# stella-cv/stella_vslam

Measured on NVIDIA H100. Metric: frames/sec (ORB+match+local BA) @1920x1080, 2000 kpts, higher is better.
Workload: dtype u8

## Files before the change

### stella_vslam_b200/csrc/lba_kernels.cu

```cuda
#include <algorithm>
#include <cmath>
#include <cstdlib>
#include <new>
#include <sched.h>

#include <chrono>
#include <memory>
#include <mutex>
#include <thread>
#include <vector>

#include "common.cuh"
#include "lm_common.cuh"
#include "quat.cuh"
#include "staging.cuh"
#include "track_chain.cuh"

namespace b200 {
namespace lba {

constexpr double kPi = 3.14159265358979323846;

struct Cam {
    int model;
// ... 302 lines not shown
        for (int j = lane; j < i; j += 32) s += W.pose_cnt[j];
#pragma unroll
        for (int d = 16; d > 0; d >>= 1) s += __shfl_down_sync(0xFFFFFFFFu, s, d);
        if (lane == 0) {
            s_start = s;
            W.pose_start[i] = s;
            if (i == W.Kf - 1) W.pose_start[W.Kf] = s + W.pose_cnt[i];
        }
    }
    __syncthreads();
    int run = s_start;
    for (int base = 0; base < W.E; base += kListThreads) {
        const int s = base + tid;
        const bool mine = s < W.E && W.epcol[s] == i;
        const unsigned bal = __ballot_sync(0xFFFFFFFFu, mine);
        if (lane == 0) warp_cnt[warp] = __popc(bal);
        __syncthreads();
        int off = 0, tot = 0;
#pragma unroll
        for (int w2 = 0; w2 < kListThreads / 32; ++w2) {
            const int c = warp_cnt[w2];
            if (w2 < warp) off += c;
            tot += c;
        }
        if (mine) {
            const int slot = run + off + __popc(bal & ((1u << lane) - 1u));
            W.pose_edges[slot] = s;
            const EdgeS* ed = W.edges + s;
            const int l = ed->point, c_lo = W.pt_start[l];
            W.rowrec[slot] = make_int4(s, ed->lcol >= 0 ? l : -1, c_lo, W.pt_start[l + 1] - c_lo);
        }
        run += tot;
        __syncthreads();
    }
}

constexpr int kSchurChunk = 64;
struct SchurBlock {
    int i, j, chunk_start, chunk_end;
};
struct SchurChunk {
    int start, end, diag, block;
};
__device__ __forceinline__ void block_to_ij(int b, int Kf, int& i, int& j) {
    const double t = 2.0 * Kf + 1.0;
    i = (int)((t - sqrt(t * t - 8.0 * b)) * 0.5);
    i = max(0, min(i, Kf - 1));
    while (i > 0 && i * Kf - i * (i - 1) / 2 > b) --i;
    while (i + 1 < Kf && (i + 1) * Kf - (i + 1) * i / 2 <= b) ++i;
    j = i + (b - (i * Kf - i * (i - 1) / 2));
}
template <bool EMIT>
__global__ void __launch_bounds__(128) plan_pairs_kernel(const WinDev* __restrict__ wins) {
    const WinDev& W = wins[blockIdx.y];
    const int lane = threadIdx.x & 31, b = blockIdx.x * 4 + (threadIdx.x >> 5);
    if (b >= W.n_blocks || *W.bad_input) return;
    int i, j;
    block_to_ij(b, W.Kf, i, j);
    const int a_lo = W.pose_start[i], a_hi = W.pose_start[i + 1], mw = W.mask_words;
    int run = EMIT ? W.blk_pair_start[b] : 0;
    for (int base = a_lo; base < a_hi; base += 32) {
        const int pos = base + lane;
        bool hit = false;
        int4 rec = make_int4(0, -1, 0, 0);
        if (pos < a_hi) {
            rec = W.rowrec[pos];
            if (rec.y >= 0) hit = (W.lm_mask[(size_t)rec.y * mw + (j >> 6)] >> (j & 63)) & 1ull;
        }
        const unsigned bal = __ballot_sync(0xFFFFFFFFu, hit);
        if (EMIT && hit) {
            int c = rec.z;
            for (int q = 0; q < rec.w; ++q)
                if (W.epcol[rec.z + q] == j) {
                    c = rec.z + q;
                    break;
                }
            W.pairs[run + __popc(bal & ((1u << lane) - 1u))] = make_int4(rec.x, c, W.pt_col[rec.y], 0);
        }
        run += __popc(bal);
    }
    if (!EMIT) {
        if (lane == 0) W.blk_cnt[b] = run;
        return;
    }
    const int ps = W.blk_pair_start[b], total = W.blk_pair_start[b + 1] - ps, cs = W.blk_chunk_start[b];
    for (int ch = lane; ch * kSchurChunk < total; ch += 32)
        W.chunks[cs + ch] = SchurChunk{ps + ch * kSchurChunk, ps + min(total, (ch + 1) * kSchurChunk), i == j ? 1 : 0, b};
    if (lane == 0) W.blocks[b] = SchurBlock{i, j, cs, W.blk_chunk_start[b + 1]};
}
__global__ void __launch_bounds__(1024) plan_pair_scan_kernel(const WinDev* __restrict__ wins) {
    const WinDev& W = wins[blockIdx.x];
    if (*W.bad_input) return;
    __shared__ int ws_p[32], ws_c[32];
    const int tid = threadIdx.x, lane = tid & 31, warp = tid >> 5, nb = W.n_blocks;
    int carry_p = 0, carry_c = 0;
    for (int base = 0; base < nb; base += 1024) {
        const int b = base + tid;
        const int vp = b < nb ? W.blk_cnt[b] : 0, vc = ceil_div(vp, kSchurChunk);
        int xp = vp, xc = vc;
#pragma unroll
        for (int d = 1; d < 32; d <<= 1) {
            const int yp = __shfl_up_sync(0xFFFFFFFFu, xp, d), yc = __shfl_up_sync(0xFFFFFFFFu, xc, d);
            if (lane >= d) {
                xp += yp;
                xc += yc;
            }
        }
        if (lane == 31) {
            ws_p[warp] = xp;
            ws_c[warp] = xc;
        }
        __syncthreads();
        if (warp == 0) {
            int sp = ws_p[lane], sc = ws_c[lane];
#pragma unroll
            for (int d = 1; d < 32; d <<= 1) {
                const int yp = __shfl_up_sync(0xFFFFFFFFu, sp, d), yc = __shfl_up_sync(0xFFFFFFFFu, sc, d);
                if (lane >= d) {
                    sp += yp;
                    sc += yc;
                }
            }
            ws_p[lane] = sp;
            ws_c[lane] = sc;
        }
        __syncthreads();
        if (b < nb) {
            W.blk_pair_start[b] = carry_p + (warp ? ws_p[warp - 1] : 0) + xp - vp;
            W.blk_chunk_start[b] = carry_c + (warp ? ws_c[warp - 1] : 0) + xc - vc;
        }
        carry_p += ws_p[31];
        carry_c += ws_c[31];
        __syncthreads();
    }
    if (tid == 0) {
        W.blk_pair_start[nb] = carry_p;
        W.blk_chunk_start[nb] = carry_c;
    }
}

__device__ double ordered_sum(const double* __restrict__ p, int n, double* stage) {
    double s = 0.0;
    for (int base = 0; base < n; base += 1024) {
        const int m = min(1024, n - base);
        __syncthreads();
        for (int i = threadIdx.x; i < m; i += blockDim.x) stage[i] = __ldcg(p + base + i);
        __syncthreads();
        if (threadIdx.x == 0)
            for (int i = 0; i < m; ++i) s += stage[i];
    }
    return s;
}

__device__ void compute_dinv(const WinDev& W, double lambda) {
    const int Lf = W.Lf;
    const double* __restrict__ Hll = W.Hll;
    double* __restrict__ Dinv = W.Dinv;
    for (int lc = threadIdx.x; lc < Lf; lc += blockDim.x) {
        const double A0 = __ldcg(Hll + lc) + lambda, A1 = __ldcg(Hll + (size_t)Lf + lc), A2 = __ldcg(Hll + (size_t)2 * Lf + lc);
        const double A4 = __ldcg(Hll + (size_t)3 * Lf + lc) + lambda, A5 = __ldcg(Hll + (size_t)4 * Lf + lc), A8 = __ldcg(Hll + (size_t)5 * Lf + lc) + lambda;
        const double c0 = A4 * A8 - A5 * A5, c1 = A5 * A2 - A1 * A8, c2 = A1 * A5 - A4 * A2;
        const double det = A0 * c0 + A1 * c1 + A2 * c2;
        if (det == 0.0 || !isfinite(det)) {
            *W.fail = 1;
            continue;
        }
        const double id = 1.0 / det;
        Dinv[lc] = c0 * id;
        Dinv[(size_t)Lf + lc] = c1 * id;
        Dinv[(size_t)2 * Lf + lc] = c2 * id;
        Dinv[(size_t)3 * Lf + lc] = (A0 * A8 - A2 * A2) * id;
        Dinv[(size_t)4 * Lf + lc] = (A1 * A2 - A0 * A5) * id;
        Dinv[(size_t)5 * Lf + lc] = (A0 * A4 - A1 * A1) * id;
    }
}

__global__ void lm_round_begin_kernel(const WinDev* __restrict__ wins, int n_windows, int iterations, int round, double gain_thr) {
    const int w = blockIdx.x * blockDim.x + threadIdx.x;
    if (w >= n_windows) return;
    LmCtl* c = wins[w].ctl;
    c->round = round;
    c->iterations = iterations;
    c->gain_thr = gain_thr;
    c->iters_done[round] = 0;
    c->need_build = 1;
    if (*wins[w].bad_input) {
        c->skip_round2 = 1;
        c->outer_go = 0;
        return;
    }
    if (round == 1 && c->abort_word && lm_aborted(c)) {
        c->skip_round2 = 1;
        c->outer_go = 0;
        return;
    }
    c->stop_flag = 0;
    c->it = 0;
    c->ok = 1;
    c->outer_go = (iterations > 0 && !(c->abort_word && *c->abort_word)) ? 1 : 0;
}

__device__ void lm_after_build(const WinDev& W, double* stage) {
    LmCtl* c = W.ctl;
    const bool first = c->it == 0;
    double chi = 0.0;
    if (first) chi = ordered_sum(W.r_chi, W.lbc, stage);
    if (threadIdx.x == 0) {
        if (first) {
            c->current_chi = chi;
            double mx = 0.0;
            for (int i = 0; i < W.lbc; ++i) mx = fmax(mx, __ldcg(W.r_diag + i));
            for (int p = 0; p < W.Kf; ++p)
                for (int a = 0; a < 6; ++a) mx = fmax(mx, fabs(__ldcg(W.Hpp + 36 * (size_t)p + a * 7)));
            c->lambda = 1e-5 * mx;
            c->ni = 2.0;
            if (c->round == 0) c->lambda_init = c->lambda;
        }
        c->qmax = 0;
        c->rho = 0.0;
        c->need_build = 0;
        *W.fail = 0;
    }
    __syncthreads();
    compute_dinv(W, c->lambda);
}

__device__ void lm_after_trial(const WinDev& W, double* stage) {
    LmCtl* c = W.ctl;
    const double* r_result = W.r_result;
    const bool ok2 = __ldcg(r_result) != 0.0;
    const double chi_sum = ordered_sum(W.r_chi, W.lbc, stage);
    const double scale_sum = ordered_sum(W.r_scale, W.lbc, stage);
    __shared__ int s_again;
    if (threadIdx.x == 0) {
        c->trials += 1;
        const double temp_chi = ok2 ? chi_sum : 1.7976931348623157e308;
        double rho = c->current_chi - temp_chi;
        double scale = ok2 ? __ldcg(r_result + 1) + scale_sum : 0.0;
        scale += 1e-3;
        rho /= scale;
        bool broke = false;
        if (rho > 0 && isfinite(temp_chi) && ok2) {
            double alpha = 1. - pow(2 * rho - 1, 3.0);
            alpha = fmin(alpha, 2. / 3.);
            c->lambda *= fmax(1. / 3., alpha);
            c->ni = 2.0;
            c->current_chi = temp_chi;
            c->cur ^= 1;
        } else {
            c->lambda *= c->ni;
            c->ni *= 2.0;
            if (!isfinite(c->lambda)) broke = true;
        }
        if (!broke) c->qmax++;
        c->rho = rho;
        const bool again = !broke && rho < 0 && c->qmax < 10 && !lm_aborted(c);
        s_again = again ? 1 : 0;
        *W.fail = 0;
        if (!again) {
            if (c->qmax == 10 || rho == 0 || !isfinite(c->lambda)) c->ok = 0;
            const double chi_now = c->current_chi;
            if (c->it == 0) {
                c->last_chi = chi_now;
            } else {
                const double gain = (c->last_chi - chi_now) / chi_now;
                c->last_chi = chi_now;
                if (gain >= 0 && gain < c->gain_thr) c->stop_flag = 1;
            }
            c->chi2[c->round] = chi_now;
            c->lambda_final[c->round] = c->lambda;
            c->it++;
            c->iters_done[c->round] = c->it;
            c->need_build = 1;
            c->outer_go = (c->it < c->iterations && !lm_aborted(c) && c->ok) ? 1 : 0;
        }
    }
    __syncthreads();
    if (s_again) compute_dinv(W, c->lambda);
}

__device__ __forceinline__ bool last_cta_arrives(int* ticket, int n_ctas, int* smem_flag) {
    __threadfence();
    __syncthreads();
    if (threadIdx.x == 0) {
        const int t = atomicAdd(ticket, 1);
        *smem_flag = (t == n_ctas - 1);
        if (*smem_flag) *ticket = 0;
    }
    __syncthreads();
    const bool last = *smem_flag != 0;
    if (last) __threadfence();
    return last;
}

__global__ void __launch_bounds__(256) lm_round_end_kernel(const WinDev* __restrict__ wins, int round) {
    __shared__ double stage[1024];
    const WinDev& W = wins[blockIdx.x];
    LmCtl* c = W.ctl;
    if (*W.bad_input || (round == 1 && c->skip_round2)) return;
    const double chi = ordered_sum(W.r_chi, W.lbc, stage);
    if (threadIdx.x) return;
    if (c->iters_done[round] == 0) c->chi2[round] = chi;
}

enum { kBuild = 0, kTrial = 1, kRoundEnd = 2 };
constexpr int kLmThreads = 128;

template <int MODE>
__global__ void __launch_bounds__(kLmThreads, 4) landmark_kernel(const WinDev* __restrict__ wins) {
    __shared__ double sh[kLmThreads];
    const WinDev& W = wins[blockIdx.y];
    if ((int)blockIdx.x >= W.lbc) return;
    const LmCtl* ctl = W.ctl;
    if (MODE == kBuild && !(ctl->outer_go && ctl->need_build)) return;
    if (MODE == kTrial && !ctl->outer_go) return;
    if (MODE == kRoundEnd && (*W.bad_input || (ctl->round == 1 && ctl->skip_round2))) return;
    const int sidx = (ctl->cur ^ (MODE == kTrial ? 1 : 0)) & 1;
    const double* __restrict__ Rt = W.Rt[sidx];
    const double* __restrict__ pts = W.pts[sidx];
    double* __restrict__ chi = W.chi[sidx];
    const double* __restrict__ chi_carry = W.chi[sidx ^ 1];
    const int sub = threadIdx.x & 7;
    const int l = blockIdx.x * 16 + (threadIdx.x >> 3);
    const bool valid = l < W.L;
    const int a0 = valid ? W.pt_start[l] : 0, b0 = valid ? W.pt_start[l + 1] : 0;
    const int lc = valid ? W.pt_col[l] : -1;
    double cost = 0.0;
    double h[9] = {0, 0, 0, 0, 0, 0, 0, 0, 0};
    double P[3] = {0, 0, 0};
    if (valid) {
        P[0] = pts[3 * (size_t)l];
        P[1] = pts[3 * (size_t)l + 1];
        P[2] = pts[3 * (size_t)l + 2];
    }
    for (int e = a0 + sub; e < b0; e += 8) {
        const EdgeS ed = W.edges[e];
        double* __restrict__ rec = W.Hpl + (size_t)e * kHplStride;
        if (W.level[e] == 0) {
            const Cam c = W.cams[ed.cam];
            double err[3], pc[3];
            const double* T = Rt + 12 * (size_t)ed.pose;
            edge_residual(ed, c, T, P, err, pc);
            const double w = (double)ed.inv_sigma_sq;
            const double e2 = w * (err[0] * err[0] + err[1] * err[1] + err[2] * err[2]);
            chi[e] = e2;
            const bool rob = W.robust[e] != 0;
            cost += rob ? huber_cost(e2, (double)ed.delta) : e2;
            if (MODE == kBuild) {
                double Ji[9], Jj[18];
                edge_jacobians(ed, c, T, pc, Ji, Jj);
                const double ww = w * (rob ? huber_weight(e2, (double)ed.delta) : 1.0);
                const bool lfree = lc >= 0, pfree = ed.pcol >= 0;
                if (lfree) {
                    h[0] += ww * (Ji[0] * Ji[0] + Ji[3] * Ji[3] + Ji[6] * Ji[6]);
                    h[1] += ww * (Ji[0] * Ji[1] + Ji[3] * Ji[4] + Ji[6] * Ji[7]);
                    h[2] += ww * (Ji[0] * Ji[2] + Ji[3] * Ji[5] + Ji[6] * Ji[8]);
                    h[3] += ww * (Ji[1] * Ji[1] + Ji[4] * Ji[4] + Ji[7] * Ji[7]);
                    h[4] += ww * (Ji[1] * Ji[2] + Ji[4] * Ji[5] + Ji[7] * Ji[8]);
                    h[5] += ww * (Ji[2] * Ji[2] + Ji[5] * Ji[5] + Ji[8] * Ji[8]);
                    h[6] += -ww * (Ji[0] * err[0] + Ji[3] * err[1] + Ji[6] * err[2]);
                    h[7] += -ww * (Ji[1] * err[0] + Ji[4] * err[1] + Ji[7] * err[2]);
                    h[8] += -ww * (Ji[2] * err[0] + Ji[5] * err[1] + Ji[8] * err[2]);
                }
                const bool both = lfree && pfree;
                double hr[12];
#pragma unroll
                for (int a = 0; a < 3; ++a)
#pragma unroll
                    for (int b = 0; b < 3; ++b) {
                        const double s = ww * (Jj[3 + a] * Ji[b] + Jj[9 + a] * Ji[3 + b] + Jj[15 + a] * Ji[6 + b]);
                        hr[a * 3 + b] = both ? s : 0.0;
                    }
#pragma unroll
                for (int i = 0; i < 3; ++i) hr[9 + i] = both ? pc[i] : 0.0;
#pragma unroll
                for (int i = 0; i < 3; ++i) st256(rec + 4 * i, hr[4 * i], hr[4 * i + 1], hr[4 * i + 2], hr[4 * i + 3]);
            }
        } else if (MODE == kBuild) {
#pragma unroll
            for (int i = 0; i < 3; ++i) st256(rec + 4 * i, 0.0, 0.0, 0.0, 0.0);
        } else if (MODE == kTrial) {
            chi[e] = chi_carry[e];
        }
    }
    if (MODE == kBuild) {
#pragma unroll
        for (int i = 0; i < 9; ++i)
#pragma unroll
            for (int s = 4; s > 0; s >>= 1) h[i] += __shfl_down_sync(0xFFFFFFFFu, h[i], s, 8);
        double mx = 0.0;
        if (valid && sub == 0 && lc >= 0) {
            const int Lf = W.Lf;
#pragma unroll
            for (int i = 0; i < 6; ++i) W.Hll[(size_t)i * Lf + lc] = h[i];
#pragma unroll
            for (int i = 0; i < 3; ++i) W.bl[(size_t)i * Lf + lc] = h[6 + i];
            mx = fmax(fabs(h[0]), fmax(fabs(h[3]), fabs(h[5])));
        }
        sh[threadIdx.x] = mx;
        __syncthreads();
        for (int s = blockDim.x >> 1; s > 0; s >>= 1) {
            if (threadIdx.x < s) sh[threadIdx.x] = fmax(sh[threadIdx.x], sh[threadIdx.x + s]);
            __syncthreads();
        }
        if (threadIdx.x == 0) W.r_diag[blockIdx.x] = sh[0];
        __syncthreads();
    }
    const double s = block_sum(cost, sh);
    if (threadIdx.x == 0) W.r_chi[blockIdx.x] = s;
    if (MODE == kTrial) {
        __shared__ int last_flag;
        __shared__ double stage[1024];
        if (!last_cta_arrives(W.tickets + 1, W.lbc, &last_flag)) return;
        lm_after_trial(W, stage);
    }
}

constexpr int kRowThreads = 256;
__global__ void __launch_bounds__(kRowThreads) pose_rows_kernel(const WinDev* __restrict__ wins) {
    const WinDev& W = wins[blockIdx.y];
    const LmCtl* ctl = W.ctl;
    if (!(ctl->outer_go && ctl->need_build)) return;
    const int n_rows = max(W.Kf, 1);
    if ((int)blockIdx.x >= n_rows) return;
    __shared__ double part[kRowThreads / 32][27];
    __shared__ int last_flag;
    __shared__ double stage[1024];
    const int tid = threadIdx.x, lane = tid & 31, warp = tid >> 5;
    if ((int)blockIdx.x < W.Kf) {
        const int i = blockIdx.x;
        const double* __restrict__ Rt = W.Rt[ctl->cur & 1];
        const double* __restrict__ pts = W.pts[ctl->cur & 1];
        const int a = W.pose_start[i], b = W.pose_start[i + 1];
        const int per = round_up(ceil_div(max(b - a, 1), kRowThreads / 32), 32);
        const int lo = a + warp * per, hi = min(b, lo + per);
        double acc[27];
#pragma unroll
        for (int x = 0; x < 27; ++x) acc[x] = 0.0;
        for (int k = lo + lane; k < hi; k += 32) {
            const int e = W.pose_edges[k];
            if (W.level[e]) continue;
            const EdgeS ed = W.edges[e];
            const Cam c = W.cams[ed.cam];
            double err[3], pc[3], Ji[9], Jj[18];
            const double* T = Rt + 12 * (size_t)ed.pose;
            edge_residual(ed, c, T, pts + 3 * (size_t)ed.point, err, pc);
            edge_jacobians(ed, c, T, pc, Ji, Jj);
            const double w = (double)ed.inv_sigma_sq;
            const double e2 = w * (err[0] * err[0] + err[1] * err[1] + err[2] * err[2]);
            const double ww = w * (W.robust[e] ? huber_weight(e2, (double)ed.delta) : 1.0);
            int t = 0;
#pragma unroll
            for (int x = 0; x < 6; ++x)
#pragma unroll
                for (int y = x; y < 6; ++y) acc[t++] += ww * (Jj[x] * Jj[y] + Jj[6 + x] * Jj[6 + y] + Jj[12 + x] * Jj[12 + y]);
#pragma unroll
            for (int x = 0; x < 6; ++x) acc[21 + x] += -ww * (Jj[x] * err[0] + Jj[6 + x] * err[1] + Jj[12 + x] * err[2]);
        }
#pragma unroll
        for (int x = 0; x < 27; ++x)
#pragma unroll
            for (int s = 16; s > 0; s >>= 1) acc[x] += __shfl_down_sync(0xFFFFFFFFu, acc[x], s);
        if (lane == 0)
#pragma unroll
            for (int x = 0; x < 27; ++x) part[warp][x] = acc[x];
        __syncthreads();
        if (tid < 27) {
            double r = 0.0;
#pragma unroll
            for (int w2 = 0; w2 < kRowThreads / 32; ++w2) r += part[w2][tid];
            if (tid < 21) {
                int x = 0, rem = tid;
                while (rem >= 6 - x) {
                    rem -= 6 - x;
                    ++x;
                }
                const int y = x + rem;
                W.Hpp[(size_t)i * 36 + x * 6 + y] = r;
                W.Hpp[(size_t)i * 36 + y * 6 + x] = r;
            } else {
                W.bp[(size_t)i * 6 + (tid - 21)] = r;
            }
        }
    }
    if (!last_cta_arrives(W.tickets, n_rows, &last_flag)) return;
    lm_after_build(W, stage);
}

__device__ __forceinline__ void dmma_m8n8k4(double& c0, double& c1, double a, double b) {
    asm volatile("mma.sync.aligned.m8n8k4.row.col.f64.f64.f64.f64 {%0,%1}, {%2}, {%3}, {%0,%1};" : "+d"(c0), "+d"(c1) : "d"(a), "d"(b));
}

__device__ __forceinline__ void schur_finish_block(const WinDev& W, const SchurBlock sb, double lambda, int lane) {
    const double* __restrict__ partials = W.chunk_part;
    double* __restrict__ M = W.M;
    const int n = W.n, ld = W.ld;
    for (int el = lane; el < 42; el += 32) {
        if (el >= 36 && sb.i != sb.j) continue;
        double sacc = 0.0;
        for (int c = sb.chunk_start; c < sb.chunk_end; ++c) sacc += __ldcg(partials + (size_t)c * 42 + el);
        if (el < 36) {
            const int r = el / 6, c = el - r * 6;
            double val = -sacc;
            if (sb.i == sb.j) val += W.Hpp[(size_t)sb.i * 36 + el] + (r == c ? lambda : 0.0);
            M[(size_t)(6 * sb.j + c) * ld + 6 * sb.i + r] = val;
            if (sb.i == sb.j) M[(size_t)(6 * sb.i + r) * ld + 6 * sb.j + c] = val;
        } else {
            const int r = el - 36;
            M[(size_t)n * ld + 6 * sb.i + r] = W.bp[(size_t)sb.i * 6 + r] - sacc;
        }
    }
}

__device__ void se3_oplus(const double* q, const double* t, const double* upd, double* qo, double* to) {
    const double* om = upd;
    const double* up = upd + 3;
    const double theta = sqrt(om[0] * om[0] + om[1] * om[1] + om[2] * om[2]);
    const double O[9] = {0, -om[2], om[1], om[2], 0, -om[0], -om[1], om[0], 0};
    double O2[9];
    for (int i = 0; i < 3; ++i)
        for (int j = 0; j < 3; ++j) O2[i * 3 + j] = O[i * 3] * O[j] + O[i * 3 + 1] * O[3 + j] + O[i * 3 + 2] * O[6 + j];
    double a, b, c, d;
    if (theta < 0.00001) {
        a = 1.0; b = 0.5; c = 0.5; d = 1.0 / 6.0;
    } else {
        a = sin(theta) / theta;
        b = (1 - cos(theta)) / (theta * theta);
        c = b;
        d = (theta - sin(theta)) / (theta * theta * theta);
    }
    double R[9], V[9];
    for (int i = 0; i < 9; ++i) {
        const double I = (i % 4 == 0) ? 1.0 : 0.0;
        R[i] = I + a * O[i] + b * O2[i];
        V[i] = I + c * O[i] + d * O2[i];
    }
    double dq[4], dt[3];
    rot_to_quat(R, dq);
    quat_normalize(dq);
    for (int i = 0; i < 3; ++i) dt[i] = V[i * 3] * up[0] + V[i * 3 + 1] * up[1] + V[i * 3 + 2] * up[2];
    double uv[3] = {dq[1] * t[2] - dq[2] * t[1], dq[2] * t[0] - dq[0] * t[2], dq[0] * t[1] - dq[1] * t[0]};
    uv[0] += uv[0]; uv[1] += uv[1]; uv[2] += uv[2];
    to[0] = dt[0] + t[0] + dq[3] * uv[0] + (dq[1] * uv[2] - dq[2] * uv[1]);
    to[1] = dt[1] + t[1] + dq[3] * uv[1] + (dq[2] * uv[0] - dq[0] * uv[2]);
    to[2] = dt[2] + t[2] + dq[3] * uv[2] + (dq[0] * uv[1] - dq[1] * uv[0]);
    double nq[4];
    nq[3] = dq[3] * q[3] - dq[0] * q[0] - dq[1] * q[1] - dq[2] * q[2];
    nq[0] = dq[3] * q[0] + dq[0] * q[3] + dq[1] * q[2] - dq[2] * q[1];
    nq[1] = dq[3] * q[1] + dq[1] * q[3] + dq[2] * q[0] - dq[0] * q[2];
    nq[2] = dq[3] * q[2] + dq[2] * q[3] + dq[0] * q[1] - dq[1] * q[0];
    quat_normalize(nq);
    qo[0] = nq[0]; qo[1] = nq[1]; qo[2] = nq[2]; qo[3] = nq[3];
}

constexpr int kCholThreads = 512;
constexpr int kNB = 24;
constexpr int kCholCluster = 8;

__device__ __forceinline__ unsigned cluster_ctarank() {
    unsigned r;
    asm volatile("mov.u32 %0, %%cluster_ctarank;" : "=r"(r));
    return r;
}
__device__ __forceinline__ unsigned cluster_nctarank() {
    unsigned r;
    asm volatile("mov.u32 %0, %%cluster_nctarank;" : "=r"(r));
    return r;
}
__device__ __forceinline__ void cluster_sync_all() {
    asm volatile("barrier.cluster.arrive.release.aligned;\n\tbarrier.cluster.wait.acquire.aligned;" ::: "memory");
}

// ... 851 lines not shown
        if (tid == 0) {
            pose_rt(q_cur, t_cur, Rt);
            s_bad = 0;
        }
        __syncthreads();
        int bad = 0;
        for (int e = tid; e < n; e += kPoseThreads) {
            const PoseEdge pe = edges[e];
            EdgeS ed;
            ed.ox = pe.ox; ed.oy = pe.oy; ed.oxr = pe.oxr;
            double err[3], pc[3];
            edge_residual(ed, cam, Rt, pe.pw, err, pc);
            const double e2 = (double)pe.inv_sigma_sq * (err[0] * err[0] + err[1] * err[1] + err[2] * err[2]);
            const double thr = (pe.oxr < 0.f) ? (double)5.99146f : (double)7.81473f;
            const unsigned char o = thr < e2 ? 1 : 0;
            flags[e] = o;
            level[e] = o;
            bad += o;
        }
        atomicAdd(&s_bad, bad);
        if (trials != 0 && trial + 1 == trials_robust) robust_on = false;
        __syncthreads();
        bad_total = s_bad;
        __syncthreads();
        if (n - bad_total < 5) break;
    }
    if (tid == 0) {
        n_valid_out[blockIdx.x] = (unsigned)(n - bad_total);
        double Rm[9];
        quat_to_rot(q_cur, Rm);
        double* M = pose_out + 16 * (size_t)blockIdx.x;
        M[0] = Rm[0]; M[1] = Rm[1]; M[2] = Rm[2]; M[3] = t_cur[0];
        M[4] = Rm[3]; M[5] = Rm[4]; M[6] = Rm[5]; M[7] = t_cur[1];
        M[8] = Rm[6]; M[9] = Rm[7]; M[10] = Rm[8]; M[11] = t_cur[2];
        M[12] = 0; M[13] = 0; M[14] = 0; M[15] = 1;
    }
}


struct Solver {
    int device = 0;
    cudaStream_t stream = nullptr;
    cudaEvent_t ev0 = nullptr, ev1 = nullptr;
    StagingArena arena;
    double* h_res = nullptr;
    size_t h_res_cap = 0;
    float last_ms = 0.f;
    int last_launches = 0;
    cudaEvent_t ev_sync = nullptr;
    cudaEvent_t ev_ctl[2] = {nullptr, nullptr};
    int* h_abort = nullptr;
    int* d_abort = nullptr;
    int abort_cap = 0;
    bool profile = false;
    std::vector<cudaEvent_t> prof_ev;
    std::vector<int> prof_kind;
    float prof_ms[8] = {};
    int prof_n[8] = {};
    bool force_offchip = false;
    int chol_cluster = kCholCluster;
    bool chol_cluster_pinned = false;
    bool last_gain_stop = false;
    int wait_mode = 3;
    cudaError_t wait(cudaStream_t st) {
        if (wait_mode == 0) return cudaStreamSynchronize(st);
        if (wait_mode >= 2) {
            cudaError_t e;
            while ((e = cudaStreamQuery(st)) == cudaErrorNotReady) {
                if (wait_mode == 2) sched_yield();
                else std::this_thread::sleep_for(std::chrono::microseconds(15));
            }
            return e;
        }
        cudaError_t e = cudaEventRecord(ev_sync, st);
        return e != cudaSuccess ? e : cudaEventSynchronize(ev_sync);
    }
    cudaError_t wait_event(cudaEvent_t ev) {
        if (wait_mode < 2) return cudaEventSynchronize(ev);
        cudaError_t e;
        while ((e = cudaEventQuery(ev)) == cudaErrorNotReady) {
            if (wait_mode == 2) sched_yield();
            else std::this_thread::sleep_for(std::chrono::microseconds(15));
        }
        return e;
    }

    int ensure_res(size_t res_doubles) {
        if (res_doubles > h_res_cap) {
            if (h_res) B200_CUDA(cudaFreeHost(h_res));
            h_res = nullptr;
            h_res_cap = 0;
            B200_CUDA(cudaHostAlloc(&h_res, sizeof(double) * res_doubles * 2, cudaHostAllocDefault));
            h_res_cap = res_doubles * 2;
        }
        return B200_OK;
    }
    int ensure_abort(int n) {
        if (n <= abort_cap) return B200_OK;
        if (h_abort) B200_CUDA(cudaFreeHost(h_abort));
        h_abort = nullptr;
        abort_cap = 0;
        B200_CUDA(cudaHostAlloc((void**)&h_abort, sizeof(int) * (size_t)n * 2, cudaHostAllocMapped));
        B200_CUDA(cudaHostGetDevicePointer((void**)&d_abort, h_abort, 0));
        abort_cap = n * 2;
        return B200_OK;
    }
};

struct WinOff {
    size_t cams, e_pose, e_point, e_cam, e_robust, e_can, e_obs, e_isig, e_delta, pose_col, pt_col, q0, t0, Rt0, pts0;
    size_t pt_cnt, pose_cnt, level, chi0, fail, tickets, bad, blk_done;
    size_t pt_start, order, edges, epcol, pose_start, pose_edges, rowrec, lm_mask, blk_cnt, blk_pair_start, blk_chunk_start, pairs, blocks, chunks,
        chunk_part, robust, q1, t1, Rt1, pts1, chi1, Hpl, Hll, bl, Dinv, Hpp, bp, M, xp, r_chi,
        r_diag, r_scale, r_result, gP, gD, ginvd;
    size_t exp_begin, qf, tf, pf, out, exp_end;
};

static int solve_batch(Solver& S, int n_all, const b200_lba_problem_t* Ps, int iters1, int iters2, volatile uint8_t* const* stops,
                       double* const* pose_outs, double* const* points_outs, uint8_t* const* outlier_outs, b200_lba_stats_t* stats, int* status, int rounds = 2, double gain_thr = 1e-3, bool allow_large = false) {
    B200_RANGE("b200:lba:batch");
    const bool debug = getenv("B200_LBA_DEBUG") != nullptr;
    const auto t_begin = std::chrono::steady_clock::now();
    auto ms_since = [](std::chrono::steady_clock::time_point t) { return std::chrono::duration<double, std::milli>(std::chrono::steady_clock::now() - t).count(); };
    std::vector<int> act;
    int ret = B200_OK;
    for (int w = 0; w < n_all; ++w) {
        if (stats) std::memset(&stats[w], 0, sizeof(stats[w]));
        status[w] = B200_OK;
        if (stops && stops[w] && *stops[w]) {
            status[w] = B200_ERR_ABORTED;
            continue;
        }
        int n_free = 0;
        for (int k = 0; k < Ps[w].n_poses; ++k) n_free += Ps[w].pose_fixed[k] ? 0 : 1;
        if (6 * n_free > (allow_large ? kCholGlobalMax : kCholOnChipMax)) {
            set_error("b200_lba_solve: window %d has %d free keyframes; the limit of this entry point is %d", w, n_free,
                      (allow_large ? kCholGlobalMax : kCholOnChipMax) / 6);
            status[w] = B200_ERR_INVALID;
            ret = B200_ERR_INVALID;
            continue;
        }
        act.push_back(w);
    }
    const int nw = (int)act.size();
    S.last_ms = 0.f;
    S.last_launches = 0;
    if (nw == 0) return ret;
    struct HostWin {
        int K, L, E, Kf, Lf, n, ld, lbc, mask_words, n_blocks, n_chunks_bound;
        size_t n_pairs;
        std::vector<int> pose_col, pt_col;
    };
    std::vector<HostWin> hw(nw);
    int maxE = 1, maxL = 1, maxKf = 1, maxK = 1, max_n = 0, max_lbc = 1, max_blocks = 1, max_chunk_warps = 1;
    std::vector<int> deg;
    for (int x = 0; x < nw; ++x) {
        const b200_lba_problem_t& P = Ps[act[x]];
        HostWin& h = hw[x];
        h.K = P.n_poses; h.L = P.n_points; h.E = P.n_edges;
        h.pose_col.resize(std::max(h.K, 1));
        h.pt_col.resize(std::max(h.L, 1));
        h.Kf = h.Lf = 0;
        for (int k = 0; k < h.K; ++k) h.pose_col[k] = P.pose_fixed[k] ? -1 : h.Kf++;
        if (P.point_fixed) {
            for (int l = 0; l < h.L; ++l) h.pt_col[l] = P.point_fixed[l] ? -1 : h.Lf++;
        } else {
            for (int l = 0; l < h.L; ++l) h.pt_col[l] = l;
            h.Lf = h.L;
        }
        h.n = 6 * h.Kf;
        h.ld = h.n + 2;
        h.lbc = std::max(1, ceil_div(h.L, 16));
        h.mask_words = std::max(1, ceil_div(h.Kf, 64));
        h.n_blocks = h.Kf * (h.Kf + 1) / 2;
        h.n_pairs = 0;
        deg.assign(std::max(h.L, 1), 0);
        for (int e = 0; e < h.E; ++e) {
            const int p = P.e_point[e], k = P.e_pose[e];
            if (p >= 0 && p < h.L && k >= 0 && k < h.K && h.pose_col[k] >= 0 && h.pt_col[p] >= 0) deg[p]++;
        }
        for (int l = 0; l < h.L; ++l) h.n_pairs += (size_t)deg[l] * (deg[l] + 1) / 2;
        h.n_chunks_bound = (int)(h.n_pairs / kSchurChunk) + h.n_blocks + 1;
        max_blocks = std::max(max_blocks, h.n_blocks);
        max_chunk_warps = std::max(max_chunk_warps, h.n_chunks_bound + h.n_blocks);
        maxE = std::max(maxE, h.E); maxL = std::max(maxL, h.L); maxKf = std::max(maxKf, h.Kf); maxK = std::max(maxK, h.K);
        max_n = std::max(max_n, h.n); max_lbc = std::max(max_lbc, h.lbc);
    }
    std::vector<WinOff> wo(nw);
    Layout cv;
    const size_t o_wins = cv.take<WinDev>(nw), o_ctl = cv.take<LmCtl>(nw);
    for (int x = 0; x < nw; ++x) {
        const HostWin& h = hw[x];
        const b200_lba_problem_t& P = Ps[act[x]];
        WinOff& o = wo[x];
        const size_t E = h.E, K = h.K, L = h.L;
        o.cams = cv.take<Cam>(P.n_cams); o.e_pose = cv.take<int>(E); o.e_point = cv.take<int>(E); o.e_cam = cv.take<unsigned char>(E);
        o.e_robust = cv.take<unsigned char>(E); o.e_can = cv.take<unsigned char>(E); o.e_obs = cv.take<float>(3 * E); o.e_isig = cv.take<float>(E);
        o.e_delta = cv.take<float>(E); o.pose_col = cv.take<int>(K); o.pt_col = cv.take<int>(L); o.q0 = cv.take<double>(4 * K);
        o.t0 = cv.take<double>(3 * K); o.Rt0 = cv.take<double>(12 * K); o.pts0 = cv.take<double>(3 * L);
    }
    const size_t upload_bytes = cv.end;
    for (int x = 0; x < nw; ++x) {
        const HostWin& h = hw[x];
        WinOff& o = wo[x];
        o.pt_cnt = cv.take<int>(h.L); o.pose_cnt = cv.take<int>(h.Kf); o.level = cv.take<unsigned char>(h.E); o.chi0 = cv.take<double>(h.E);
        o.fail = cv.take<int>(1); o.tickets = cv.take<int>(2); o.bad = cv.take<int>(1); o.blk_done = cv.take<int>(h.n_blocks);
    }
    const size_t zero_end = cv.end;
    for (int x = 0; x < nw; ++x) {
        const HostWin& h = hw[x];
        WinOff& o = wo[x];
        const size_t E = h.E, K = h.K, L = h.L, Kf = h.Kf, Lf = h.Lf;
        o.pt_start = cv.take<int>(L + 1); o.order = cv.take<int>(E); o.edges = cv.take<EdgeS>(E); o.epcol = cv.take<int>(E);
        o.pose_start = cv.take<int>(Kf + 1); o.pose_edges = cv.take<int>(E); o.rowrec = cv.take<int4>(E);
        o.lm_mask = cv.take<unsigned long long>(L * (size_t)h.mask_words); o.blk_cnt = cv.take<int>(h.n_blocks);
        o.blk_pair_start = cv.take<int>(h.n_blocks + 1); o.blk_chunk_start = cv.take<int>(h.n_blocks + 1); o.pairs = cv.take<int4>(h.n_pairs);
        o.blocks = cv.take<SchurBlock>(h.n_blocks); o.chunks = cv.take<SchurChunk>(h.n_chunks_bound);
        o.chunk_part = cv.take<double>(42 * (size_t)h.n_chunks_bound); o.robust = cv.take<unsigned char>(E);
        o.q1 = cv.take<double>(4 * K); o.t1 = cv.take<double>(3 * K); o.Rt1 = cv.take<double>(12 * K); o.pts1 = cv.take<double>(3 * L);
        o.chi1 = cv.take<double>(E); o.Hpl = cv.take<double>(kHplStride * E); o.Hll = cv.take<double>(6 * Lf); o.bl = cv.take<double>(3 * Lf);
        o.Dinv = cv.take<double>(6 * Lf); o.Hpp = cv.take<double>(36 * Kf); o.bp = cv.take<double>(6 * Kf);
        o.M = cv.take<double>((size_t)(h.n + 1) * h.ld); o.xp = cv.take<double>(h.n);
        o.gP = o.gD = o.ginvd = 0;
        if (h.n > kCholOnChipMax || S.force_offchip) {
            o.gP = cv.take<double>((size_t)kNB * ((h.n + 1 + 3) & ~3));
            o.gD = cv.take<double>(kNB * (kNB + 1));
            o.ginvd = cv.take<double>(h.n);
        }
        o.r_chi = cv.take<double>(h.lbc); o.r_diag = cv.take<double>(h.lbc); o.r_scale = cv.take<double>(h.lbc); o.r_result = cv.take<double>(8);
    }
    const size_t export_begin = cv.end;
    for (int x = 0; x < nw; ++x) {
        const HostWin& h = hw[x];
        WinOff& o = wo[x];
        o.qf = cv.take<double>(4 * (size_t)h.K); o.tf = cv.take<double>(3 * (size_t)h.K); o.pf = cv.take<double>(3 * (size_t)h.L);
        o.out = cv.take<unsigned char>(h.E);
    }
    const size_t export_bytes = cv.end - export_begin;
    const size_t ctl_doubles = ceil_div(sizeof(LmCtl) * (size_t)nw, sizeof(double)) + 8;
    int rc = S.arena.reserve(cv.end + 512, upload_bytes, S.stream);
    if (rc) return rc;
    if ((rc = S.ensure_res(ceil_div(export_bytes, sizeof(double)) + 2 * ctl_doubles + 64))) return rc;
    if ((rc = S.ensure_abort(nw))) return rc;
    unsigned char* d = S.arena.d;
    unsigned char* hs = S.arena.h;
    LmCtl* h_ctl2[2] = {reinterpret_cast<LmCtl*>(S.h_res), reinterpret_cast<LmCtl*>(S.h_res + ctl_doubles)};
    LmCtl* h_ctl = h_ctl2[0];
    unsigned char* h_export = reinterpret_cast<unsigned char*>(S.h_res + 2 * ctl_doubles + 8);
    WinDev* hwd = reinterpret_cast<WinDev*>(hs + o_wins);
    LmCtl* hctl0 = reinterpret_cast<LmCtl*>(hs + o_ctl);
    for (int x = 0; x < nw; ++x) {
        const HostWin& h = hw[x];
        const b200_lba_problem_t& P = Ps[act[x]];
        const WinOff& o = wo[x];
        const size_t E = h.E, K = h.K, L = h.L;
        Cam* cams = reinterpret_cast<Cam*>(hs + o.cams);
        for (int i = 0; i < P.n_cams; ++i) {
            const b200_camera_t& c = P.cams[i];
            cams[i] = Cam{c.model, c.fx, c.fy, c.cx, c.cy, c.fxb, c.cols, c.rows};
        }
        if (E) {
            std::memcpy(hs + o.e_pose, P.e_pose, sizeof(int) * E);
            std::memcpy(hs + o.e_point, P.e_point, sizeof(int) * E);
            std::memcpy(hs + o.e_cam, P.e_cam, E);
            if (P.e_robust) std::memcpy(hs + o.e_robust, P.e_robust, E);
            else std::memset(hs + o.e_robust, 1, E);
            if (P.e_can_be_outlier) std::memcpy(hs + o.e_can, P.e_can_be_outlier, E);
            else std::memset(hs + o.e_can, 1, E);
            std::memcpy(hs + o.e_obs, P.e_obs, sizeof(float) * 3 * E);
            std::memcpy(hs + o.e_isig, P.e_inv_sigma_sq, sizeof(float) * E);
            std::memcpy(hs + o.e_delta, P.e_delta, sizeof(float) * E);
        }
        if (K) std::memcpy(hs + o.pose_col, h.pose_col.data(), sizeof(int) * K);
        if (L) {
            std::memcpy(hs + o.pt_col, h.pt_col.data(), sizeof(int) * L);
            std::memcpy(hs + o.pts0, P.points, sizeof(double) * 3 * L);
        }
        double* q0 = reinterpret_cast<double*>(hs + o.q0);
        double* t0 = reinterpret_cast<double*>(hs + o.t0);
        double* Rt0 = reinterpret_cast<double*>(hs + o.Rt0);
        for (size_t k = 0; k < K; ++k) {
            const double* M = P.pose_cw + 16 * k;
            const double R[9] = {M[0], M[1], M[2], M[4], M[5], M[6], M[8], M[9], M[10]};
            rot_to_quat(R, &q0[4 * k]);
            quat_normalize(&q0[4 * k]);
            t0[3 * k] = M[3]; t0[3 * k + 1] = M[7]; t0[3 * k + 2] = M[11];
            quat_to_rot(&q0[4 * k], &Rt0[12 * k]);
            Rt0[12 * k + 9] = M[3]; Rt0[12 * k + 10] = M[7]; Rt0[12 * k + 11] = M[11];
        }
        WinDev& W = hwd[x];
        std::memset(&W, 0, sizeof(W));
        W.K = h.K; W.L = h.L; W.E = h.E; W.Kf = h.Kf; W.Lf = h.Lf; W.n = h.n; W.ld = h.ld; W.n_cams = P.n_cams; W.lbc = h.lbc;
        W.e_pose = (const int*)(d + o.e_pose); W.e_point = (const int*)(d + o.e_point); W.e_cam = d + o.e_cam; W.e_robust = d + o.e_robust;
        W.e_can_outlier = d + o.e_can; W.e_obs = (const float*)(d + o.e_obs); W.e_isig = (const float*)(d + o.e_isig);
        W.e_delta = (const float*)(d + o.e_delta); W.pose_col = (const int*)(d + o.pose_col); W.pt_col = (const int*)(d + o.pt_col);
        W.cams = (const Cam*)(d + o.cams);
        W.pt_cnt = (int*)(d + o.pt_cnt); W.pt_start = (int*)(d + o.pt_start); W.order = (int*)(d + o.order); W.edges = (EdgeS*)(d + o.edges);
        W.epcol = (int*)(d + o.epcol); W.pose_cnt = (int*)(d + o.pose_cnt); W.pose_start = (int*)(d + o.pose_start);
        W.pose_edges = (int*)(d + o.pose_edges); W.level = d + o.level; W.robust = d + o.robust;
        W.rowrec = (int4*)(d + o.rowrec);
        W.lm_mask = (unsigned long long*)(d + o.lm_mask); W.mask_words = h.mask_words; W.n_blocks = h.n_blocks; W.blk_cnt = (int*)(d + o.blk_cnt);
        W.blk_pair_start = (int*)(d + o.blk_pair_start); W.blk_chunk_start = (int*)(d + o.blk_chunk_start); W.pairs = (int4*)(d + o.pairs);
        W.blocks = (SchurBlock*)(d + o.blocks); W.chunks = (SchurChunk*)(d + o.chunks); W.chunk_part = (double*)(d + o.chunk_part);
        W.blk_done = (int*)(d + o.blk_done);
        W.q[0] = (double*)(d + o.q0); W.q[1] = (double*)(d + o.q1); W.t[0] = (double*)(d + o.t0); W.t[1] = (double*)(d + o.t1);
        W.Rt[0] = (double*)(d + o.Rt0); W.Rt[1] = (double*)(d + o.Rt1); W.pts[0] = (double*)(d + o.pts0); W.pts[1] = (double*)(d + o.pts1);
        W.chi[0] = (double*)(d + o.chi0); W.chi[1] = (double*)(d + o.chi1);
        W.Hpl = (double*)(d + o.Hpl); W.Hll = (double*)(d + o.Hll); W.bl = (double*)(d + o.bl); W.Dinv = (double*)(d + o.Dinv);
        W.Hpp = (double*)(d + o.Hpp); W.bp = (double*)(d + o.bp); W.M = (double*)(d + o.M); W.xp = (double*)(d + o.xp);
        W.gP = (double*)(d + o.gP); W.gD = (double*)(d + o.gD); W.ginvd = (double*)(d + o.ginvd);
        W.r_chi = (double*)(d + o.r_chi); W.r_diag = (double*)(d + o.r_diag); W.r_scale = (double*)(d + o.r_scale); W.r_result = (double*)(d + o.r_result);
        W.fail = (int*)(d + o.fail); W.tickets = (int*)(d + o.tickets); W.bad_input = (int*)(d + o.bad);
        W.ctl = (LmCtl*)(d + o_ctl) + x;
        W.qf = (double*)(d + o.qf); W.tf = (double*)(d + o.tf); W.pf = (double*)(d + o.pf); W.out = d + o.out;
        LmCtl& c = hctl0[x];
        std::memset(&c, 0, sizeof(c));
        c.ok = 1;
        S.h_abort[x] = 0;
        c.abort_word = (stops && stops[act[x]]) ? S.d_abort + x : nullptr;
    }
    if (debug) fprintf(stderr, "[lba] %d windows staged in %.3f ms (upload %.2f MB, arena %.1f MB)\n", nw, ms_since(t_begin), upload_bytes / 1e6, cv.end / 1e6);
    cudaStream_t st = S.stream;
    int launches = 0;
    S.prof_kind.clear();
    auto mark = [&](int kind) -> int {
        if (!S.profile) return B200_OK;
        const size_t idx = S.prof_kind.size();
        if (idx >= S.prof_ev.size()) {
            cudaEvent_t e;
            B200_CUDA(cudaEventCreate(&e));
            S.prof_ev.push_back(e);
        }
        B200_CUDA(cudaEventRecord(S.prof_ev[idx], st));
        S.prof_kind.push_back(kind);
        return B200_OK;
    };
    B200_CUDA(cudaEventRecord(S.ev0, st));
    B200_CUDA(S.arena.upload(upload_bytes, st));
    B200_CUDA(cudaMemsetAsync(d + upload_bytes, 0, zero_end - upload_bytes, st));
    if ((rc = mark(-1))) return rc;
    const WinDev* wins = (const WinDev*)(d + o_wins);
    const LmCtl* d_ctl = (const LmCtl*)(d + o_ctl);
    plan_count_kernel<<<dim3(ceil_div(maxE, 256), nw), 256, 0, st>>>(wins);
    plan_scan_kernel<<<nw, 1024, 0, st>>>(wins);
    plan_place_kernel<<<dim3(ceil_div(maxE, 256), nw), 256, 0, st>>>(wins);
    plan_sort_kernel<<<dim3(ceil_div(maxL, 128), nw), 128, 0, st>>>(wins);
    plan_pose_lists_kernel<<<dim3(maxKf, nw), kListThreads, 0, st>>>(wins);
    plan_pairs_kernel<false><<<dim3(ceil_div(max_blocks, 4), nw), 128, 0, st>>>(wins);
    plan_pair_scan_kernel<<<nw, 1024, 0, st>>>(wins);
    plan_pairs_kernel<true><<<dim3(ceil_div(max_blocks, 4), nw), 128, 0, st>>>(wins);
    launches += 8;
    if ((rc = mark(0))) return rc;
    B200_RANGE("b200:lba:rounds+export");
    const bool large = max_n > kCholOnChipMax || S.force_offchip;
    const size_t chol_smem = sizeof(double) * ((size_t)kNB * (kNB + 1) + 4 + (size_t)((std::min(max_n, kCholOnChipMax) + 1 + 3) & ~3) * kNB);
    B200_CUDA(cudaFuncSetAttribute(chol_solve_kernel, cudaFuncAttributeMaxDynamicSharedMemorySize, (int)chol_smem));
    const int chol_cluster = S.chol_cluster_pinned ? S.chol_cluster : (nw <= 2 ? 8 : 4);
    auto launch_rep = [&]() -> int {
        int rcm;
        landmark_kernel<kBuild><<<dim3(max_lbc, nw), kLmThreads, 0, st>>>(wins);
        if ((rcm = mark(1))) return rcm;
        pose_rows_kernel<<<dim3(maxKf, nw), kRowThreads, 0, st>>>(wins);
        if ((rcm = mark(2))) return rcm;
        schur_mma_kernel<<<dim3(ceil_div(max_chunk_warps, 4), nw), 128, 4 * kSmmaWarpDoubles * sizeof(double), st>>>(wins);
        if ((rcm = mark(3))) return rcm;
        if (large) {
            for (int kb = 0; kb < max_n; kb += kNB) {
                const int m = max_n + 1 - std::min(kb + kNB, max_n);
                const long long tm = (m + 3) >> 2, n_tiles = tm * (tm + 1) / 2;
                gchol_panel_kernel<<<dim3(ceil_div(m + 4, kGcholThreads), nw), kGcholThreads, 0, st>>>(wins, kb);
                gchol_trail_kernel<<<dim3((unsigned)std::max<long long>(1, (n_tiles + kGcholThreads - 1) / kGcholThreads), nw), kGcholThreads, 0, st>>>(wins, kb);
                launches += 2;
            }
            gchol_finish_kernel<<<nw, kGfinThreads, 0, st>>>(wins);
        } else {
            cudaLaunchConfig_t cfg = {};
            cfg.gridDim = dim3(chol_cluster * nw);
            cfg.blockDim = dim3(kCholThreads);
            cfg.dynamicSmemBytes = chol_smem;
            cfg.stream = st;
            cudaLaunchAttribute attr[1];
            attr[0].id = cudaLaunchAttributeClusterDimension;
            attr[0].val.clusterDim.x = chol_cluster;
            attr[0].val.clusterDim.y = 1;
            attr[0].val.clusterDim.z = 1;
            cfg.attrs = attr;
            cfg.numAttrs = 1;
            B200_CUDA(cudaLaunchKernelEx(&cfg, chol_solve_kernel, wins));
        }
        if ((rcm = mark(4))) return rcm;
        backsub_kernel<<<dim3(max_lbc, nw), 128, 0, st>>>(wins);
        if ((rcm = mark(5))) return rcm;
        launches += 5;
        return B200_OK;
    };
    auto fetch_issue = [&](int b) -> int {
        B200_CUDA(cudaMemcpyAsync(h_ctl2[b], d_ctl, sizeof(LmCtl) * nw, cudaMemcpyDeviceToHost, st));
        B200_CUDA(cudaEventRecord(S.ev_ctl[b], st));
        return B200_OK;
    };
    auto fetch_wait = [&](int b) -> int {
        B200_CUDA(S.wait_event(S.ev_ctl[b]));
        h_ctl = h_ctl2[b];
        for (int x = 0; x < nw; ++x)
            if (stops && stops[act[x]] && *stops[act[x]]) S.h_abort[x] = 1;
        return B200_OK;
    };
    auto fetch_ctl = [&]() -> int {
        int r_ = fetch_issue(0);
        return r_ ? r_ : fetch_wait(0);
    };
    const int iters[2] = {iters1, iters2};
    int rc2;
    for (int r = 0; r < rounds; ++r) {
        if (r == 1) {
            if ((rc2 = fetch_ctl())) return rc2;
            for (int x = 0; x < nw; ++x) {
                volatile uint8_t* f = stops ? stops[act[x]] : nullptr;
                if (!f) continue;
                if (h_ctl[x].stop_flag || *f) {
                    S.h_abort[x] = 1;
                    *f = 1;
                } else {
                    S.h_abort[x] = 0;
                }
            }
        }
        lm_round_begin_kernel<<<ceil_div(nw, 64), 64, 0, st>>>(wins, nw, iters[r], r, gain_thr);
        ++launches;
        if (r == 1) {
            outlier_kernel<<<dim3(ceil_div(maxE, 128), nw), 128, 0, st>>>(wins, 0);
            ++launches;
        }
        if (iters[r] > 0) {
            int need = iters[r];
            for (;;) {
                const int chunk = std::max(1, std::min(need, 6));
                for (int i = 0; i < chunk; ++i)
                    if ((rc2 = launch_rep())) return rc2;
                if ((rc2 = fetch_ctl())) return rc2;
                need = 0;
                for (int x = 0; x < nw; ++x)
                    if (h_ctl[x].outer_go) need = std::max(need, std::max(1, h_ctl[x].iterations - h_ctl[x].it));
                if (need == 0) break;
            }
        }
        landmark_kernel<kRoundEnd><<<dim3(max_lbc, nw), kLmThreads, 0, st>>>(wins);
        lm_round_end_kernel<<<nw, 256, 0, st>>>(wins, r);
        launches += 2;
    }
    if (rounds == 2) outlier_kernel<<<dim3(ceil_div(maxE, 128), nw), 128, 0, st>>>(wins, 1);
    lm_export_kernel<<<dim3(ceil_div(std::max(std::max(4 * maxK, 3 * maxL), 1), 256), nw), 256, 0, st>>>(wins);
    launches += 2;
    B200_CUDA(cudaGetLastError());
    if ((rc = mark(7))) return rc;
    B200_CUDA(cudaEventRecord(S.ev1, st));
    B200_CUDA(cudaMemcpyAsync(h_export, d + export_begin, export_bytes, cudaMemcpyDeviceToHost, st));
    std::vector<int> h_bad(nw, 0);
    if ((rc2 = fetch_ctl())) return rc2;
    for (int x = 0; x < nw; ++x) B200_CUDA(cudaMemcpyAsync(&h_bad[x], d + wo[x].bad, sizeof(int), cudaMemcpyDeviceToHost, st));
    B200_CUDA(cudaStreamSynchronize(st));
    B200_CUDA(cudaEventElapsedTime(&S.last_ms, S.ev0, S.ev1));
    S.last_launches = launches;
    for (int k2 = 0; k2 < 8; ++k2) {
        S.prof_ms[k2] = 0.f;
        S.prof_n[k2] = 0;
    }
    for (size_t m = 1; m < S.prof_kind.size(); ++m) {
        float ms = 0.f;
        B200_CUDA(cudaEventElapsedTime(&ms, S.prof_ev[m - 1], S.prof_ev[m]));
        const int kd = S.prof_kind[m];
        if (kd >= 0 && kd < 8) {
            S.prof_ms[kd] += ms;
            S.prof_n[kd] += 1;
        }
    }
    if (debug) fprintf(stderr, "[lba] batch of %d windows: %.3f ms wall, %.3f ms on the stream, %d launches\n", nw, ms_since(t_begin), S.last_ms, launches);
    for (int x = 0; x < nw; ++x) {
        const int w = act[x];
        const HostWin& h = hw[x];
        const b200_lba_problem_t& P = Ps[w];
        const WinOff& o = wo[x];
        if (h_bad[x]) {
            set_error("b200_lba_solve: edge %d of window %d references an invalid vertex/camera", h_bad[x] - 1, w);
            status[w] = B200_ERR_INVALID;
            ret = B200_ERR_INVALID;
            continue;
        }
        const LmCtl& c = h_ctl[x];
        if (stats) {
            stats[w].lambda_init = c.lambda_init;
            for (int r = 0; r < 2; ++r) {
                stats[w].iterations[r] = c.iters_done[r];
                stats[w].chi2[r] = c.chi2[r];
                stats[w].lambda_final[r] = c.lambda_final[r];
            }
        }
        if (stops && stops[w] && c.stop_flag) *stops[w] = 1;
        S.last_gain_stop = c.stop_flag != 0;
        const unsigned char* ex = h_export + (o.qf - export_begin);
        const double* qf = reinterpret_cast<const double*>(ex);
        const double* tf = reinterpret_cast<const double*>(h_export + (o.tf - export_begin));
        const double* pf = reinterpret_cast<const double*>(h_export + (o.pf - export_begin));
        const unsigned char* out = h_export + (o.out - export_begin);
        int n_out = 0;
        for (int e = 0; e < h.E && rounds == 2; ++e) n_out += out[e];
        if (rounds == 2 && outlier_outs && outlier_outs[w] && h.E) std::memcpy(outlier_outs[w], out, h.E);
        if (stats) stats[w].n_outliers = n_out;
        if (h.L) std::memcpy(points_outs[w], pf, sizeof(double) * 3 * (size_t)h.L);
        for (int k = 0; k < h.K; ++k) {
            double* M = pose_outs[w] + 16 * (size_t)k;
            if (P.pose_fixed[k]) {
                std::memcpy(M, P.pose_cw + 16 * (size_t)k, sizeof(double) * 16);
                continue;
            }
            double R[9];
            quat_to_rot(&qf[4 * k], R);
            M[0] = R[0]; M[1] = R[1]; M[2] = R[2]; M[3] = tf[3 * k];
            M[4] = R[3]; M[5] = R[4]; M[6] = R[5]; M[7] = tf[3 * k + 1];
            M[8] = R[6]; M[9] = R[7]; M[10] = R[8]; M[11] = tf[3 * k + 2];
            M[12] = 0; M[13] = 0; M[14] = 0; M[15] = 1;
        }
    }
    return ret;
}

constexpr int kTrackEdgeThreads = 256;
constexpr int kMatchedBias = 1 << 30;
__global__ void __launch_bounds__(kTrackEdgeThreads) track_edges_kernel(chain::TrackShared sh, const chain::TrackFrameDev* __restrict__ frames,
                                                                        PoseProb* __restrict__ probs, PoseEdge* __restrict__ edges_all,
                                                                        int* __restrict__ edge_kp_all, const int* __restrict__ gate) {
    __shared__ int warp_sum[kTrackEdgeThreads / 32];
    __shared__ int s_base;
    const chain::TrackFrameDev& F = frames[blockIdx.x];
    const int tid = threadIdx.x, lane = tid & 31, warp = tid >> 5;
    const int n = F.status[0];
    int* slot = F.kp_landmark_out;
    for (int i = tid; i < F.kp_cap; i += kTrackEdgeThreads) {
        int l = -1;
        if (i < n && F.kp_landmark && i < F.n_kp_in) {
            l = F.kp_landmark[i];
            if (l < 0 || l >= F.n_lm) l = -1;
        }
        slot[i] = l;
        F.kp_outlier[i] = 0;
    }
// ... 366 lines not shown
```

Before: 10100.

## Move landmark Dinv computation into a grid-parallel kernel before Schur

Replaces the single-CTA compute_dinv, which ran in the last-arriving block after the chi reduction and after each trial, with a separate grid-wide kernel launched before schur_mma. The work is spread across many CTAs instead of one serial block at the end of the reduction. It also adds a min-blocks hint of 2 to pose_rows_kernel's launch bounds. The trade is one more kernel launch per LM repetition. There is also a risk: when a trial is rejected and lambda changes, Dinv is now only recomputed on the next launch_rep, not right after the trial, so the retry path must rebuild it correctly.

```diff
diff --git a/stella_vslam_b200/csrc/lba_kernels.cu b/stella_vslam_b200/csrc/lba_kernels.cu
--- a/stella_vslam_b200/csrc/lba_kernels.cu
+++ b/stella_vslam_b200/csrc/lba_kernels.cu
@@ -478,27 +478,30 @@
     return s;
 }
 
-__device__ void compute_dinv(const WinDev& W, double lambda) {
-    const int Lf = W.Lf;
+constexpr int kDinvThreads = 256;
+__global__ void __launch_bounds__(kDinvThreads) landmark_dinv_kernel(const WinDev* __restrict__ wins) {
+    const WinDev& W = wins[blockIdx.y];
+    const LmCtl* __restrict__ ctl = W.ctl;
+    const int Lf = W.Lf, lc = blockIdx.x * kDinvThreads + threadIdx.x;
+    if (lc >= Lf || !ctl->outer_go) return;
+    const double lambda = ctl->lambda;
     const double* __restrict__ Hll = W.Hll;
     double* __restrict__ Dinv = W.Dinv;
-    for (int lc = threadIdx.x; lc < Lf; lc += blockDim.x) {
-        const double A0 = __ldcg(Hll + lc) + lambda, A1 = __ldcg(Hll + (size_t)Lf + lc), A2 = __ldcg(Hll + (size_t)2 * Lf + lc);
-        const double A4 = __ldcg(Hll + (size_t)3 * Lf + lc) + lambda, A5 = __ldcg(Hll + (size_t)4 * Lf + lc), A8 = __ldcg(Hll + (size_t)5 * Lf + lc) + lambda;
-        const double c0 = A4 * A8 - A5 * A5, c1 = A5 * A2 - A1 * A8, c2 = A1 * A5 - A4 * A2;
-        const double det = A0 * c0 + A1 * c1 + A2 * c2;
-        if (det == 0.0 || !isfinite(det)) {
-            *W.fail = 1;
-            continue;
-        }
-        const double id = 1.0 / det;
-        Dinv[lc] = c0 * id;
-        Dinv[(size_t)Lf + lc] = c1 * id;
-        Dinv[(size_t)2 * Lf + lc] = c2 * id;
-        Dinv[(size_t)3 * Lf + lc] = (A0 * A8 - A2 * A2) * id;
-        Dinv[(size_t)4 * Lf + lc] = (A1 * A2 - A0 * A5) * id;
-        Dinv[(size_t)5 * Lf + lc] = (A0 * A4 - A1 * A1) * id;
-    }
+    const double A0 = Hll[lc] + lambda, A1 = Hll[(size_t)Lf + lc], A2 = Hll[(size_t)2 * Lf + lc];
+    const double A4 = Hll[(size_t)3 * Lf + lc] + lambda, A5 = Hll[(size_t)4 * Lf + lc], A8 = Hll[(size_t)5 * Lf + lc] + lambda;
+    const double c0 = A4 * A8 - A5 * A5, c1 = A5 * A2 - A1 * A8, c2 = A1 * A5 - A4 * A2;
+    const double det = A0 * c0 + A1 * c1 + A2 * c2;
+    if (det == 0.0 || !isfinite(det)) {
+        *W.fail = 1;
+        return;
+    }
+    const double id = 1.0 / det;
+    Dinv[lc] = c0 * id;
+    Dinv[(size_t)Lf + lc] = c1 * id;
+    Dinv[(size_t)2 * Lf + lc] = c2 * id;
+    Dinv[(size_t)3 * Lf + lc] = (A0 * A8 - A2 * A2) * id;
+    Dinv[(size_t)4 * Lf + lc] = (A1 * A2 - A0 * A5) * id;
+    Dinv[(size_t)5 * Lf + lc] = (A0 * A4 - A1 * A1) * id;
 }
 
 __global__ void lm_round_begin_kernel(const WinDev* __restrict__ wins, int n_windows, int iterations, int round, double gain_thr) {
@@ -547,8 +550,6 @@
         c->need_build = 0;
         *W.fail = 0;
     }
-    __syncthreads();
-    compute_dinv(W, c->lambda);
 }
 
 __device__ void lm_after_trial(const WinDev& W, double* stage) {
@@ -557,7 +558,6 @@
     const bool ok2 = __ldcg(r_result) != 0.0;
     const double chi_sum = ordered_sum(W.r_chi, W.lbc, stage);
     const double scale_sum = ordered_sum(W.r_scale, W.lbc, stage);
-    __shared__ int s_again;
     if (threadIdx.x == 0) {
         c->trials += 1;
         const double temp_chi = ok2 ? chi_sum : 1.7976931348623157e308;
@@ -581,7 +581,6 @@
         if (!broke) c->qmax++;
         c->rho = rho;
         const bool again = !broke && rho < 0 && c->qmax < 10 && !lm_aborted(c);
-        s_again = again ? 1 : 0;
         *W.fail = 0;
         if (!again) {
             if (c->qmax == 10 || rho == 0 || !isfinite(c->lambda)) c->ok = 0;
@@ -601,8 +600,6 @@
             c->outer_go = (c->it < c->iterations && !lm_aborted(c) && c->ok) ? 1 : 0;
         }
     }
-    __syncthreads();
-    if (s_again) compute_dinv(W, c->lambda);
 }
 
 __device__ __forceinline__ bool last_cta_arrives(int* ticket, int n_ctas, int* smem_flag) {
@@ -743,7 +740,7 @@
 }
 
 constexpr int kRowThreads = 256;
-__global__ void __launch_bounds__(kRowThreads) pose_rows_kernel(const WinDev* __restrict__ wins) {
+__global__ void __launch_bounds__(kRowThreads, 2) pose_rows_kernel(const WinDev* __restrict__ wins) {
     const WinDev& W = wins[blockIdx.y];
     const LmCtl* ctl = W.ctl;
     if (!(ctl->outer_go && ctl->need_build)) return;
@@ -1901,7 +1898,7 @@
         std::vector<int> pose_col, pt_col;
     };
     std::vector<HostWin> hw(nw);
-    int maxE = 1, maxL = 1, maxKf = 1, maxK = 1, max_n = 0, max_lbc = 1, max_blocks = 1, max_chunk_warps = 1;
+    int maxE = 1, maxL = 1, max_Lf = 1, maxKf = 1, maxK = 1, max_n = 0, max_lbc = 1, max_blocks = 1, max_chunk_warps = 1;
     std::vector<int> deg;
     for (int x = 0; x < nw; ++x) {
         const b200_lba_problem_t& P = Ps[act[x]];
@@ -1932,7 +1929,7 @@
         h.n_chunks_bound = (int)(h.n_pairs / kSchurChunk) + h.n_blocks + 1;
         max_blocks = std::max(max_blocks, h.n_blocks);
         max_chunk_warps = std::max(max_chunk_warps, h.n_chunks_bound + h.n_blocks);
-        maxE = std::max(maxE, h.E); maxL = std::max(maxL, h.L); maxKf = std::max(maxKf, h.Kf); maxK = std::max(maxK, h.K);
+        maxE = std::max(maxE, h.E); maxL = std::max(maxL, h.L); max_Lf = std::max(max_Lf, h.Lf); maxKf = std::max(maxKf, h.Kf); maxK = std::max(maxK, h.K);
         max_n = std::max(max_n, h.n); max_lbc = std::max(max_lbc, h.lbc);
     }
     std::vector<WinOff> wo(nw);
@@ -2111,6 +2108,7 @@
         if ((rcm = mark(1))) return rcm;
         pose_rows_kernel<<<dim3(maxKf, nw), kRowThreads, 0, st>>>(wins);
         if ((rcm = mark(2))) return rcm;
+        landmark_dinv_kernel<<<dim3(ceil_div(max_Lf, kDinvThreads), nw), kDinvThreads, 0, st>>>(wins);
         schur_mma_kernel<<<dim3(ceil_div(max_chunk_warps, 4), nw), 128, 4 * kSmmaWarpDoubles * sizeof(double), st>>>(wins);
         if ((rcm = mark(3))) return rcm;
         if (large) {
@@ -2140,7 +2138,7 @@
         if ((rcm = mark(4))) return rcm;
         backsub_kernel<<<dim3(max_lbc, nw), 128, 0, st>>>(wins);
         if ((rcm = mark(5))) return rcm;
-        launches += 5;
+        launches += 6;
         return B200_OK;
     };
     auto fetch_issue = [&](int b) -> int {
```

Measured after the change: 10280 (median of 6 runs). No clear change (+1.7%).
